# juicedata/juicefs

Measured on AMD Instinct MI355X. Metric: device-resident GiB/s (de)compress, 4 MiB blocks, LZ4+Zstd, 1/2/4/8 MI355X, higher is better.
Workload: dtype u8; 1 GPU; LZ4 decompress, 4096x4MiB blocks already in HBM (BASELINE configs[1]); blocks_per_gpu=4096, block_bytes=4194304, class=T, compressed_bytes_per_gpu=8570049795, parallelism=1 process(es), one per GPU, blocks sharded, no collective

## Files before the change

### juicefs_amd/csrc/lz4_decode.hip

```cpp
#include <hip/hip_runtime.h>
#include <stdint.h>

#include "jfs_internal.h"
#include "lz4_put16.h"
#include "lz4_tailpack.h"
#include "wave.cuh"

namespace jfs {
namespace lz4d {

constexpr int P = 32;
constexpr int CW = 64 * P;
constexpr int CWIN = CW + 80;
constexpr int R = 4096;
constexpr int RMASK = R - 1;
constexpr int SEG = 128;
constexpr int TMAX = CW / 3 + 2;
constexpr int TCAP = 448 < TMAX ? 448 : TMAX;
#ifndef JFS_DIAG
#define JFS_DIAG 0
#endif
enum : unsigned {
    D_SKIP_ZERO = 1,
    D_SKIP_LIT = 2,
    D_SKIP_FAR = 4,
    D_SKIP_SUBST = 8,
    D_SKIP_NEAR = 16,
    D_PARSEONLY = 32,
    D_NOCOPY = 64,
};
constexpr unsigned DIAG = JFS_DIAG;
constexpr uint32_t STOP = 0x80000000u;
constexpr uint32_t NONE = 0xFFFFFFFFu;
constexpr int KEXT = 64;
constexpr int FLUSH_T = 1024;
constexpr int LMAX = 64;
constexpr int BSPAN = 2048;
static_assert(BSPAN + FLUSH_T + 128 <= R, "ring must hold the unflushed tail plus one batch");
static_assert(R - BSPAN >= LMAX + 16, "far sources must lie below the flushed prefix");
static_assert(R == (int)TP_RING && LMAX <= (int)TP_LEN_MAX, "tail_pack field widths (lz4_tailpack.h)");

#ifdef JFS_PROF
#define NPROF 20
__device__ uint64_t g_prof[NPROF];
struct Prof {
    uint64_t t, acc[NPROF];
    __device__ void start() {
        t = __builtin_amdgcn_s_memtime();
        for (int i = 0; i < NPROF; i++) acc[i] = 0;
    }
    __device__ void stamp(int k) {
        uint64_t x = __builtin_amdgcn_s_memtime();
        acc[k] += x - t;
        t = x;
    }
    __device__ void flush_out() {
        if (__lane_id() == 0)
            for (int i = 0; i < NPROF; i++) atomicAdd((unsigned long long *)&g_prof[i], acc[i]);
    }
};
#define PSTAMP(k) pr.stamp(k)
#define PCOUNT(k, n) (pr.acc[k] += (n))
#define PROF_ARG , Prof &pr
#define PROF_PASS , pr
#else
#define PSTAMP(k)
#define PCOUNT(k, n)
#define PROF_ARG
#define PROF_PASS
#endif

enum { W_NONE = 0, W_WIN = 1, W_SER = 2, W_BUG = 3 };
struct Meta {
    int32_t kind, wbase, cbase;
    uint32_t T, efin;
};
struct Ctl {
    int32_t done, restart, rip;
    int32_t step;
};

struct Smem {
    alignas(16) uint8_t ring[R];
    alignas(16) uint8_t cwin[2][CWIN];
    alignas(16) uint16_t tab[2][TCAP];
    Meta meta[2];
    Ctl ctl;
};

struct Ctx {
    const gc_u8 *src;
    g_u8 *dst;
    int32_t n;
    int32_t cap;
    int32_t F;
    int32_t Fw;
    uint32_t dmis;
    int32_t cbase;
    int32_t bug;
    uint8_t *cw;
    uint32_t cwoff;
    uint16_t *tab;
};

typedef uint32_t u32x4 __attribute__((ext_vector_type(4), aligned(4)));
typedef uint32_t u32x2 __attribute__((ext_vector_type(2), aligned(4)));
typedef JFS_GLOBAL const u32x4 gc_x4;
typedef JFS_GLOBAL const u32x2 gc_x2;

__device__ __forceinline__ uint32_t slot(const Ctx &c, int32_t pos) { return (uint32_t)(pos + (int32_t)c.dmis) & RMASK; }

template <bool UNDER>
__device__ __forceinline__ void far_load(const Ctx &c, uintptr_t a, uint32_t &d0, uint32_t &d1, uint32_t &d2,
                                         uint32_t &d3, uint32_t &d4, uint32_t &d5) {
    const uintptr_t b = a & ~(uintptr_t)3, lo = (uintptr_t)c.dst & ~(uintptr_t)3;
    const bool under = UNDER && b < lo;
    const gc_x4 *q = (const gc_x4 *)(under ? lo : b);
    const u32x4 v = q[0];
    const u32x2 w = *(const gc_x2 *)(q + 1);
    d0 = v.x; d1 = v.y; d2 = v.z; d3 = v.w; d4 = w.x; d5 = w.y;
    if (under) { d5 = d4; d4 = d3; d3 = d2; d2 = d1; d1 = d0; d0 = 0; }
}

__device__ __forceinline__ uint32_t cb(const Smem &s, const Ctx &c, int32_t p) {
    int32_t r = p - c.cbase;
    if ((uint32_t)r < (uint32_t)CWIN) return c.cw[r];
    return (p >= 0 && p < c.n) ? c.src[p] : 0u;
}

__device__ __forceinline__ void stage_window(Smem &s, Ctx &c, int32_t wbase) {
    const int l = lane_id();
    const uint32_t mis = (uint32_t)(((uintptr_t)c.src + (uint32_t)wbase) & 15u);
    c.cbase = wbase - (int32_t)mis;
    constexpr int NCH = (CWIN / 16 + 63) / 64;
    uint4 v[NCH];
#pragma unroll
    for (int j = 0; j < NCH; ++j) {
        const int k = l + 64 * j;
        const int32_t p = c.cbase + 16 * k;
        v[j] = make_uint4(0, 0, 0, 0);
        if (k < CWIN / 16 && p < c.n) v[j] = *(const gc_u4 *)(c.src + p);
    }
#pragma unroll
    for (int j = 0; j < NCH; ++j) {
        const int k = l + 64 * j;
        if (k < CWIN / 16) *(uint4 *)(c.cw + 16 * k) = v[j];
    }
    if (c.cbase < 0 || c.cbase + CWIN > c.n) {
        for (int k = l; k < CWIN; k += 64) {
            int32_t p = c.cbase + k;
            if (p >= c.n || p < 0) c.cw[k] = 0;
        }
    }
}

struct Tok {
    int32_t nxt;
    int32_t ll;
    int32_t ml;
    int32_t off;
    int32_t lit;
    int32_t llx;
};

__device__ __forceinline__ Tok parse_tok(const Smem &s, const Ctx &c, int32_t p) {
    Tok t;
    const int32_t n = c.n;
    t.ll = t.ml = t.off = t.lit = t.llx = 0;
    if (p > n - 18) { t.nxt = (int32_t)(STOP | (uint32_t)p); return t; }
    uint32_t tb = cb(s, c, p);
    int32_t q = p + 1;
    int32_t ll = (int32_t)(tb >> 4);
    if (ll == 15) {
        t.llx = 1;
        int k = 0;
        uint32_t sv;
        do {
            sv = cb(s, c, q);
            q++;
            ll += (int32_t)sv;
            if (q >= n - 15 || ++k > KEXT) { t.nxt = (int32_t)(STOP | (uint32_t)p); return t; }
        } while (sv == 255);
        if (q + ll > n - 32) { t.nxt = (int32_t)(STOP | (uint32_t)p); return t; }
    }
    t.lit = q;
    t.ll = ll;
    q += ll;
    t.off = (int32_t)(cb(s, c, q) | (cb(s, c, q + 1) << 8));
    q += 2;
    int32_t ml = (int32_t)(tb & 15);
    if (ml == 15) {
        int k = 0;
        uint32_t sv;
        do {
            sv = cb(s, c, q);
            q++;
            ml += (int32_t)sv;
            if (q >= n - 4 || ++k > KEXT) { t.nxt = (int32_t)(STOP | (uint32_t)p); return t; }
        } while (sv == 255);
    }
    t.ml = ml + 4;
    t.nxt = q;
    return t;
}

struct FTok {
    int32_t nxt, lit;
    uint32_t ll, ml, off, llx;
    bool slow, stop;
};

__device__ __forceinline__ uint32_t w8(const Ctx &c, int32_t r) { return c.cw[r < CWIN - 1 ? r : CWIN - 1]; }

__device__ __forceinline__ FTok parse_fast(const Smem &s, const Ctx &c, int32_t p) {
    FTok t;
    const int32_t n = c.n, b0 = c.cbase;
    const int32_t r = p - b0;
    const uint32_t tb = w8(c, r), e1 = w8(c, r + 1);
    const bool llx = (tb >> 4) == 15;
    int32_t q = r + 1 + (llx ? 1 : 0);
    t.ll = (tb >> 4) + (llx ? e1 : 0u);
    bool slow = llx && e1 == 255;
    bool stop = p > n - 18;
    stop |= llx && (b0 + q >= n - 15 || b0 + q + (int32_t)t.ll > n - 32);
    t.lit = b0 + q;
    q += (int32_t)t.ll;
    slow |= q + 3 > CWIN;
    const uint32_t o0 = w8(c, q), o1 = w8(c, q + 1), e2 = w8(c, q + 2);
    q += 2;
    const bool mlx = (tb & 15) == 15;
    t.ml = (tb & 15) + (mlx ? e2 : 0u) + 4;
    q += mlx ? 1 : 0;
    slow |= mlx && e2 == 255;
    stop |= mlx && b0 + q >= n - 4;
    t.off = o0 | (o1 << 8);
    t.llx = llx ? 1u : 0u;
    t.nxt = b0 + q;
    t.slow = slow;
    t.stop = stop;
    return t;
}

__device__ __forceinline__ void flush(Smem &s, Ctx &c, int32_t to) {
    const int l = lane_id();
    int32_t F = c.F;
    if (to <= F) return;
    int32_t a = F + (int32_t)((16u - ((c.dmis + (uint32_t)F) & 15u)) & 15u);
    if (a > to) a = to;
    if (l < a - F) c.dst[F + l] = s.ring[slot(c, F + l)];
    int32_t b = a + ((to - a) & ~15);
    for (int32_t x = a + 16 * l; x < b; x += 1024) {
        uint4 v = *(const uint4 *)(s.ring + slot(c, x));
        *(g_u4 *)(c.dst + x) = v;
    }
    if (l < to - b) c.dst[b + l] = s.ring[slot(c, b + l)];
    c.F = to;
}

__device__ __forceinline__ void flush_to_line(Smem &s, Ctx &c, int32_t hi) {
    int32_t to = (int32_t)(((uint32_t)hi + c.dmis) & ~127u) - (int32_t)c.dmis;
    if (to > c.F) flush(s, c, to);
}

__device__ __forceinline__ uint32_t out_byte(const Smem &s, const Ctx &c, int32_t x, int32_t ringfloor) {
    if (x >= ringfloor) return s.ring[slot(c, x)];
    return c.dst[x];
}

__device__ __forceinline__ void need_flushed(Ctx &c, int32_t lim) {
    if (lim > c.Fw) {
        wait_vm();
        c.Fw = c.F;
    }
}

constexpr int32_t LIT_DIRECT = 2 * R;
__device__ __forceinline__ void direct_lit(Smem &s, Ctx &c, int32_t srcpos, int32_t op, int32_t body) {
    const int l = lane_id();
    flush(s, c, op);
    const gc_u8 *sp = c.src + srcpos - op;
    int32_t x = op;
    const int32_t ha = (int32_t)((16u - (((uint32_t)(uintptr_t)(c.dst + x)) & 15u)) & 15u);
    if (l < ha) c.dst[x + l] = sp[x + l];
    x += ha;
    for (; x + 4096 <= body; x += 4096) {
        u32x4 v[4];
        uint32_t w[4];
        const uint32_t sh = (uint32_t)((uintptr_t)(sp + x) & 3u);
#pragma unroll
        for (int j = 0; j < 4; ++j) {
            const uintptr_t a = (uintptr_t)(sp + x + 1024 * j + 16 * l) & ~(uintptr_t)3;
            v[j] = *(const gc_x4 *)a;
            w[j] = *(const gc_u32 *)(a + 16);
        }
#pragma unroll
        for (int j = 0; j < 4; ++j) {
            uint4 o;
            o.x = __builtin_amdgcn_alignbyte(v[j].y, v[j].x, sh);
            o.y = __builtin_amdgcn_alignbyte(v[j].z, v[j].y, sh);
            o.z = __builtin_amdgcn_alignbyte(v[j].w, v[j].z, sh);
            o.w = __builtin_amdgcn_alignbyte(w[j], v[j].w, sh);
            *(g_u4 *)(c.dst + x + 1024 * j + 16 * l) = o;
        }
    }
    for (; x < body; x += 64)
        if (x + l < body) c.dst[x + l] = sp[x + l];
    c.F = body;
}

__device__ __forceinline__ void coop_lit(Smem &s, Ctx &c, int32_t srcpos, int32_t op, int32_t len) {
    int l = lane_id();
    asm volatile("" : "+v"(l));
    if (len >= LIT_DIRECT) {
        const int32_t body = op + len - R;
        direct_lit(s, c, srcpos, op, body);
        srcpos += body - op;
        len -= body - op;
        op = body;
    }
    for (int32_t k = 0; k < len; k += 64) {
        if (op + k - c.F >= FLUSH_T) flush_to_line(s, c, op + k);
        int32_t i = k + l;
        if (i < len) s.ring[slot(c, op + i)] = cb(s, c, srcpos + i);
    }
}

__device__ __forceinline__ int32_t direct_fill(Smem &s, Ctx &c, int32_t op, int32_t off, int32_t len) {
    const int l = lane_id();
    const int32_t body = op + len - R;
    flush(s, c, op);
    const uint32_t amis = (uint32_t)(uintptr_t)(c.dst + op) & 15u;
    const int32_t x0 = op + (int32_t)((16u - amis) & 15u);
    uint32_t q[4] = {0, 0, 0, 0};
#pragma unroll
    for (int b = 0; b < 16; ++b) {
        const uint32_t v = s.ring[slot(c, op - off + (int32_t)(((uint32_t)(x0 - op) + (uint32_t)b) % (uint32_t)off))];
        q[b >> 2] |= v << (8 * (b & 3));
    }
    const uint4 chunk = make_uint4(q[0], q[1], q[2], q[3]);
    if (op + l < x0) c.dst[op + l] = s.ring[slot(c, op - off + (l % off))];
    int32_t x = x0;
    for (; x + 4096 <= body; x += 4096) {
#pragma unroll
        for (int j = 0; j < 4; ++j) *(g_u4 *)(c.dst + x + 1024 * j + 16 * l) = chunk;
    }
    for (; x + 16 <= body; x += 1024)
        if (x + 16 * l + 16 <= body) *(g_u4 *)(c.dst + x + 16 * l) = chunk;
    const int32_t xe = x0 + ((body - x0) & ~15);
    if (xe + l < body) c.dst[xe + l] = (uint8_t)(q[l >> 2 & 3] >> (8 * (l & 3)));
    if (l < 16) {
        const int32_t y = body - 16 + l;
        s.ring[slot(c, y)] = s.ring[slot(c, op - off + (int32_t)((uint32_t)(y - op) % (uint32_t)off))];
    }
    c.F = body;
    return body;
}

__device__ __forceinline__ void coop_match(Smem &s, Ctx &c, int32_t op, int32_t off, int32_t len) {
    int l = lane_id();
    asm volatile("" : "+v"(l));
    if (len >= LIT_DIRECT && off > 0 && off <= 16 && (16 % off) == 0) {
        const int32_t b = direct_fill(s, c, op, off, len);
        len -= b - op;
        op = b;
    }
    int32_t m = 0, step = 0;
    if (off > 0 && off < 64) { m = l % off; step = 64 % off; }
    for (int32_t k = 0; k < len; k += 64) {
        int32_t hi = op + k;
        if (hi - c.F >= FLUSH_T) flush_to_line(s, c, hi);
        int32_t ringfloor = hi + 64 - R;
        int32_t i = k + l;
        uint32_t v = 0;
        int32_t x = 0;
        if (off > 0) x = (off >= 64) ? op - off + i : op - off + m;
// ... 124 lines not shown
    cpy = op + length;
    if (cpy > cap - 12 && cpy > cap - 5) goto err;
    coop_match(s, c, op, offset, (int32_t)length);
    op = (int32_t)cpy;
    st.ip = ip;
    st.op = op;
    return SER_CONT;
err:
    st.ip = ip;
    st.ret = -ip - 1;
    return SER_ERR;
}

__device__ __forceinline__ uint32_t lomask(int32_t k) {
    k = k < 0 ? 0 : k;
    return k >= 4 ? 0xFFFFFFFFu : ((1u << (8 * k)) - 1u);
}

__device__ __forceinline__ void lds_or(uint8_t *ring, uint32_t a, uint32_t v) {
    __hip_atomic_fetch_or(reinterpret_cast<uint32_t *>(ring) + (a >> 2), v, __ATOMIC_RELAXED,
                          __HIP_MEMORY_SCOPE_WORKGROUP);
}
__device__ __forceinline__ void lds_or_at(uint32_t *p, uint32_t v) {
    __hip_atomic_fetch_or(p, v, __ATOMIC_RELAXED, __HIP_MEMORY_SCOPE_WORKGROUP);
}

template <bool WRAP>
__device__ __forceinline__ void put16(Smem &s, uint32_t da, int32_t m, uint32_t w0, uint32_t w1, uint32_t w2,
                                      uint32_t w3, uint32_t w4) {
    uint8_t *ring = s.ring;
    const Put16Masks k = put16_masks(da & 3u, (uint32_t)m);
    if constexpr (WRAP) {
        const uint32_t D0 = da & ~3u;
        lds_or(ring, D0, w0 & k.k[0]);
        lds_or(ring, (D0 + 4) & RMASK, w1 & k.k[1]);
        lds_or(ring, (D0 + 8) & RMASK, w2 & k.k[2]);
        lds_or(ring, (D0 + 12) & RMASK, w3 & k.k[3]);
        lds_or(ring, (D0 + 16) & RMASK, w4 & k.k[4]);
    } else {
        uint32_t *p = reinterpret_cast<uint32_t *>(ring) + (da >> 2);
        lds_or_at(p, w0 & k.k[0]);
        lds_or_at(p + 1, w1 & k.k[1]);
        lds_or_at(p + 2, w2 & k.k[2]);
        lds_or_at(p + 3, w3 & k.k[3]);
        lds_or_at(p + 4, w4 & k.k[4]);
    }
}

template <bool WRAP>
__device__ __forceinline__ void zero_span(Smem &s, const Ctx &c, int32_t O0, int32_t O1) {
    const int l = lane_id();
    const uint32_t a = slot(c, O0), h = a & 3u;
    if (l == 0 && h)
        __hip_atomic_fetch_and(reinterpret_cast<uint32_t *>(s.ring) + (a >> 2), lomask((int32_t)h), __ATOMIC_RELAXED,
                               __HIP_MEMORY_SCOPE_WORKGROUP);
    if constexpr (WRAP) {
        const int32_t A = O0 + (int32_t)((4u - h) & 3u);
        for (int32_t x = A + 4 * l; x < O1; x += 256) *(uint32_t *)(s.ring + slot(c, x)) = 0u;
    } else {
        const uint32_t e = a + (uint32_t)(O1 - O0);
        for (uint32_t x = ((a + 3u) & ~3u) + 4u * (uint32_t)l; x < e; x += 256) *(uint32_t *)(s.ring + x) = 0u;
    }
}

template <bool RING, bool WRAP>
__device__ __forceinline__ void copy16(Smem &s, uint32_t sa, uint32_t da, int32_t m) {
    const uint8_t *lds = (const uint8_t *)&s;
    const uint32_t ha = da & 3u;
    const uint32_t sb = RING ? (sa - ha) & RMASK : sa - ha, S0 = sb & ~3u, sh = sb & 3u;
    uint32_t r[6];
    if (RING && __ballot(S0 > (uint32_t)(R - 24))) {
#pragma unroll
        for (int j = 0; j < 6; ++j) r[j] = *(const uint32_t *)(lds + ((S0 + 4 * j) & RMASK));
    } else {
#pragma unroll
        for (int j = 0; j < 6; ++j) r[j] = *(const uint32_t *)(lds + S0 + 4 * j);
    }
    put16<WRAP>(s, da, m, __builtin_amdgcn_alignbyte(r[1], r[0], sh), __builtin_amdgcn_alignbyte(r[2], r[1], sh),
                __builtin_amdgcn_alignbyte(r[3], r[2], sh), __builtin_amdgcn_alignbyte(r[4], r[3], sh),
                __builtin_amdgcn_alignbyte(r[5], r[4], sh));
}


template <bool WRAP>
__device__ __forceinline__ void wave_near(Smem &s, uint32_t ds, uint32_t ss, int32_t len) {
    const int l = lane_id();
    const int32_t D = (int32_t)((ds - ss) & RMASK);
    const int32_t step = D < 64 ? D : 64;
    if (!WRAP && ss + (uint32_t)len <= (uint32_t)R) {
        const int32_t back = (int32_t)ss - (int32_t)ds;
        uint8_t *d = s.ring + ds + l;
        for (int32_t left = len; left > 0; left -= step, d += step)
            if (l < (left < step ? left : step)) d[0] = d[back];
        return;
    }
    for (int32_t k = 0; k < len; k += step) {
        const int32_t i = k + l;
        if (l < step && i < len) s.ring[(ds + (uint32_t)i) & RMASK] = s.ring[(ds + (uint32_t)(i - D)) & RMASK];
    }
}
__device__ __forceinline__ void wave_lit(Smem &s, const Ctx &c, int32_t op, uint32_t litr, int32_t from, int32_t len) {
    const int l = lane_id();
    for (int32_t k = from; k < len; k += 64) {
        const int32_t i = k + l;
        if (i < len) s.ring[slot(c, op + i)] = c.cw[litr + (uint32_t)i];
    }
}

template <bool WRAP>
__device__ __forceinline__ void batch(Smem &s, Ctx &c, bool act, int32_t o, uint32_t ll, uint32_t ml, uint32_t off,
                                      uint32_t litr, int32_t O0, int32_t O1 PROF_ARG) {
    const int32_t hz = O1 + 4 - R;
    asm volatile("" : "+v"(o));
    PCOUNT(14, 1);
    if (O0 - c.F >= FLUSH_T) flush_to_line(s, c, O0);
    if constexpr (!(DIAG & D_SKIP_ZERO)) zero_span<WRAP>(s, c, O0, O1);
    const int32_t ms = o + (int32_t)ll, msrc = ms - (int32_t)off;
    const uint32_t sbias = c.dmis - (((uint32_t)O0 + c.dmis) & ~(uint32_t)RMASK);
    auto dslot = [&](int32_t pos) -> uint32_t { return WRAP ? slot(c, pos) : (uint32_t)pos + sbias; };
    const bool hasm = act && ml > 0;
    const bool zero = hasm && off == 0;
    const bool far = hasm && off != 0 && msrc < hz;
    if (__ballot(far) && hz + LMAX > c.Fw) {
        wait_vm();
        c.Fw = c.F;
        if (hz + LMAX > c.Fw) c.bug = 4;
    }
    uint32_t fd0 = 0, fd1 = 0, fd2 = 0, fd3 = 0, fd4 = 0, fd5 = 0;
    const uint32_t fha = slot(c, ms) & 3u;
    if (__ballot(far)) {
        if (__ballot(far && msrc < 4)) {
            if (far) far_load<true>(c, (uintptr_t)(c.dst + msrc) - fha, fd0, fd1, fd2, fd3, fd4, fd5);
        } else {
            if (far) far_load<false>(c, (uintptr_t)(c.dst + msrc) - fha, fd0, fd1, fd2, fd3, fd4, fd5);
        }
    }
    for (uint32_t k = 0; !(DIAG & D_SKIP_LIT) && __ballot(act && k < ll); k += 16) {
        PCOUNT(16, 1);
        if (act && k < ll) {
            const int32_t m = ll - k < 16u ? (int32_t)(ll - k) : 16;
            copy16<false, WRAP>(s, c.cwoff + litr + k, dslot(o + (int32_t)k), m);
        }
    }
    PSTAMP(4);
    if (!(DIAG & D_SKIP_FAR) && __ballot(far)) {
        for (uint32_t k = 0; __ballot(far && k < ml); k += 16) {
            PCOUNT(17, 1);
            if (far && k < ml) {
                const int32_t m = ml - k < 16u ? (int32_t)(ml - k) : 16;
                const uint32_t da = dslot(ms + (int32_t)k);
                const uint32_t sh = (uint32_t)((uintptr_t)(c.dst + msrc + (int32_t)k) - fha) & 3u;
                put16<WRAP>(s, da, m, __builtin_amdgcn_alignbyte(fd1, fd0, sh),
                            __builtin_amdgcn_alignbyte(fd2, fd1, sh), __builtin_amdgcn_alignbyte(fd3, fd2, sh),
                            __builtin_amdgcn_alignbyte(fd4, fd3, sh), __builtin_amdgcn_alignbyte(fd5, fd4, sh));
            }
            const bool more = far && k + 16 < ml;
            if (__ballot(more)) {
                if (more)
                    far_load<false>(c, (uintptr_t)(c.dst + msrc + (int32_t)k + 16) - fha, fd0, fd1, fd2, fd3, fd4, fd5);
            }
        }
    }
    PSTAMP(5);
    bool pend = hasm && !far && !zero;
    int32_t src = msrc;
    const uint64_t am = __ballot(act);
    const int first = am ? (int)__builtin_ctzll(am) : 0;
    const uint32_t key = act ? (uint32_t)ms : (lane_id() < first ? 0u : 0xFFFFFFFFu);
    bool litsrc = false;
    {
        const uint32_t mek = pend ? (uint32_t)(ms + (int32_t)ml) : 0u;
        const bool want = !(DIAG & D_SKIP_SUBST) && pend && off >= ml && src >= O0;
        if (__ballot(want)) {
            int lo = 0;
#pragma unroll
            for (int stp = 32; stp; stp >>= 1) {
                const uint32_t v = (uint32_t)__shfl((int)key, lo + stp, 64);
                lo = v <= (uint32_t)src ? lo + stp : lo;
            }
            const uint32_t vms = (uint32_t)__shfl((int)key, lo, 64);
            const uint32_t vme = (uint32_t)__shfl((int)mek, lo, 64);
            const int32_t voff = __shfl((int)off, lo, 64);
            const bool ok = want && vms <= (uint32_t)src && (uint32_t)(src + (int32_t)ml) <= vme && voff > 0 &&
                            src - voff >= hz;
            const uint32_t nms = (uint32_t)__shfl((int)key, lo + 1 < 64 ? lo + 1 : 63, 64);
            litsrc = want && vms <= (uint32_t)src && (uint32_t)src >= vme && lo < 63 &&
                     (uint32_t)(src + (int32_t)ml) <= nms;
            src = ok ? src - voff : src;
        }
    }
    int32_t pos = ms, rem = (int32_t)ml, D = ms - src;
    const int32_t send = src + (int32_t)ml < ms ? src + (int32_t)ml : ms;
    if (!(DIAG & D_SKIP_NEAR)) {
        PCOUNT(18, 1);
        const bool go = pend && (send <= O0 || litsrc);
        if (__ballot(go)) {
            PCOUNT(15, 1);
            if (go) {
                const int32_t m = rem < 16 ? (rem < D ? rem : D) : (D < 16 ? D : 16);
                copy16<true, WRAP>(s, slot(c, pos - D), dslot(pos), m);
                pos += m;
                rem -= m;
                if (rem <= 0) pend = false;
            }
        }
        const uint32_t tw = tail_pack(dslot(pos), slot(c, pos - D), (uint32_t)rem, (uint32_t)D);
        for (uint64_t pmk = __ballot(pend); pmk;) {
            const int j = (int)__builtin_ctzll(pmk);
            pmk &= ~(1ull << j);
            PCOUNT(19, 1);
            const uint32_t w = readlane(tw, j);
            if (tail_direct(w)) {
                if ((uint32_t)lane_id() < tail_rem(w)) s.ring[tail_ds(w) + lane_id()] = s.ring[tail_ss(w) + lane_id()];
            } else {
                wave_near<WRAP>(s, tail_ds(w), tail_ss(w), (int32_t)tail_rem(w));
            }
        }
    }
    PSTAMP(6);
}

__device__ __forceinline__ uint32_t copy_tokens(Smem &s, Ctx &c, uint32_t T, int32_t op0, int32_t *end_op,
                                                int32_t *bad_ip PROF_ARG) {
    const int l = lane_id();
    int32_t op = op0;
    const int32_t cap = c.cap;
    if constexpr ((DIAG & D_PARSEONLY) != 0) {
        *end_op = op0;
        return T;
    }
    for (uint32_t g0 = 0; g0 < T; g0 += 64) {
        const uint32_t n0 = T - g0 < 64u ? T - g0 : 64u;
        const bool in0 = (uint32_t)l < n0;
        const int32_t p = c.cbase + (in0 ? (int32_t)c.tab[g0 + l] : 0);
        FTok t = parse_fast(s, c, p);
        const bool sl = in0 && t.slow;
        if (__ballot(sl)) {
            if (sl) {
                const Tok u = parse_tok(s, c, p);
                t.lit = u.lit;
                t.ll = (uint32_t)u.ll;
                t.ml = (uint32_t)u.ml;
                t.off = (uint32_t)u.off;
                t.llx = (uint32_t)u.llx;
            }
        }
        const uint32_t ll = in0 ? t.ll : 0u, ml = in0 ? t.ml : 0u, off = t.off;
        const uint32_t litr = (uint32_t)(t.lit - c.cbase);
        const uint32_t len = ll + ml;
        const uint32_t incl = dpp_scan_add(len);
        const int32_t o = op + (int32_t)(incl - len);
        const int32_t om = o + (int32_t)ll;
        const bool bad = in0 && ((t.llx && om > cap - 32) || (om + (int32_t)ml >= cap - 64) || ((int32_t)off > om));
        const uint64_t bm = __ballot(bad);
        const uint32_t n = bm ? (uint32_t)__builtin_ctzll(bm) : n0;
        const bool in = (uint32_t)l < n;
        const int32_t endo = o + (int32_t)len;
        const bool lng = in && (ll > (uint32_t)LMAX || ml > (uint32_t)LMAX);
        PSTAMP(2);
        uint32_t j = 0;
        while (j < n) {
            const int32_t oj = (int32_t)readlane((uint32_t)o, (int)j);
            if (readlane(lng ? 1u : 0u, (int)j)) {
                const uint32_t jll = readlane(ll, (int)j), jml = readlane(ml, (int)j), joff = readlane(off, (int)j);
                const uint32_t jlit = readlane(litr, (int)j);
                coop_lit(s, c, c.cbase + (int32_t)jlit, oj, (int32_t)jll);
                coop_match(s, c, oj + (int32_t)jll, (int32_t)joff, (int32_t)jml);
                PSTAMP(7);
                j++;
                continue;
            }
            const bool ok = (uint32_t)l >= j && in && !lng && endo - oj <= BSPAN;
            const uint64_t stop = __ballot(!ok) & (~0ull << j);
            const uint32_t e = stop ? (uint32_t)__builtin_ctzll(stop) : 64u;
            const uint32_t eb = e > n ? n : e;
            const bool act = (uint32_t)l >= j && (uint32_t)l < eb;
            const int32_t O1 = (int32_t)readlane((uint32_t)endo, (int)eb - 1);
            PSTAMP(3);
            if constexpr (!(DIAG & D_NOCOPY)) {
                if (slot(c, oj) + (uint32_t)(O1 - oj) + 20u <= (uint32_t)R)
                    batch<false>(s, c, act, o, ll, ml, off, litr, oj, O1 PROF_PASS);
                else
                    batch<true>(s, c, act, o, ll, ml, off, litr, oj, O1 PROF_PASS);
            }
            j = eb;
        }
        if (bm) {
            *bad_ip = (int32_t)readlane((uint32_t)p, (int)n);
            *end_op = (int32_t)readlane((uint32_t)o, (int)n);
            return g0 + n;
        }
        op += (int32_t)readlane(incl, 63);
    }
    *end_op = op;
    return T;
}

static_assert(SEG == 128, "segment bit sets are two u64 per lane");
constexpr int SW = 64 * SEG;
constexpr int SPRE = 32;
constexpr int SEG_BUDGET = 64;
constexpr int SEG_MIN = 4;

__device__ __noinline__ uint32_t g_next_exact(const Ctx &c, int32_t p) {
    const int32_t n = c.n;
    if (p > n - 18) return STOP | (uint32_t)p;
    const uint32_t tb = c.src[p];
    int32_t q = p + 1;
    int32_t ll = (int32_t)(tb >> 4);
    if (ll == 15) {
        int k = 0;
        uint32_t sv;
        do {
            sv = c.src[q];
            q++;
            ll += (int32_t)sv;
            if (q >= n - 15 || ++k > KEXT) return STOP | (uint32_t)p;
        } while (sv == 255);
        if (q + ll > n - 32) return STOP | (uint32_t)p;
    }
    q += ll + 2;
    if ((tb & 15u) == 15u) {
        int k = 0;
        uint32_t sv;
        do {
            sv = c.src[q];
            q++;
            if (q >= n - 4 || ++k > KEXT) return STOP | (uint32_t)p;
        } while (sv == 255);
    }
    return (uint32_t)q;
}

__device__ __forceinline__ uint32_t g_step(const Ctx &c, int32_t p, bool act) {
    const int32_t n = c.n;
    const uint32_t edge = (uint32_t)(p > n - 18);
    const uint32_t up = (uint32_t)p;
    const uint32_t tb = c.src[edge ? 0u : up], e1 = c.src[edge ? 0u : up + 1u];
    const uint32_t hi = tb >> 4;
    const uint32_t llx = (uint32_t)(hi == 15u);
    const uint32_t L = llx ? 15u + e1 : hi;
    const uint32_t lstop = llx & ((uint32_t)(p + 2 >= n - 15) | (uint32_t)(p + 2 + (int32_t)L > n - 32));
    const uint32_t q = up + 3u + llx + L;
    const uint32_t e2 = c.src[(edge | lstop) ? 0u : q];
    const uint32_t mlx = (uint32_t)((tb & 15u) == 15u);
    uint32_t x = q + mlx;
    const uint32_t slow = (uint32_t)act & (edge ^ 1u) & (lstop ^ 1u) & ((llx & (uint32_t)(e1 == 255u)) | (mlx & (uint32_t)(e2 == 255u)));
    x = (edge | lstop | (mlx & (uint32_t)((int32_t)x >= n - 4))) ? (STOP | up) : x;
    if (__ballot(slow)) {
        if (slow) x = g_next_exact(c, p);
    }
    return x;
}

__device__ __forceinline__ bool tbit2(uint64_t a0, uint64_t a1, uint32_t d) {
    return (((d < 64u ? a0 : a1) >> (d & 63u)) & 1ull) != 0;
}
__device__ __forceinline__ void sbit2(uint64_t &a0, uint64_t &a1, uint32_t d) {
    const uint64_t m = 1ull << (d & 63u);
    a0 |= d < 64u ? m : 0ull;
    a1 |= d < 64u ? 0ull : m;
}
__device__ __forceinline__ uint64_t from_lo(uint32_t d) { return d < 64u ? (~0ull << (d & 63u)) : 0ull; }
__device__ __forceinline__ uint64_t from_hi(uint32_t d) { return d < 64u ? ~0ull : (~0ull << (d & 63u)); }

struct SegWalk {
    int32_t base, plo, phi;
    int32_t q;
    uint32_t cur;
    uint32_t sx, ex;
    uint64_t vs0, vs1;
    uint64_t vt0, vt1;
    uint64_t vp0, vp1;
    bool mv;
    int phase;
    bool round;
    int steps, rounds;

    __device__ __forceinline__ void start(int32_t b) {
        const int l = lane_id();
        base = b;
        plo = b + l * SEG;
        phi = plo + SEG;
        cur = l == 0 ? (uint32_t)b : (uint32_t)(plo - SPRE);
        q = (int32_t)cur;
        vs0 = vs1 = vt0 = vt1 = vp0 = vp1 = 0;
        sx = ex = 0;
        mv = true;
        phase = 0;
        round = false;
        steps = rounds = 0;
    }

    __device__ __forceinline__ bool advance(Ctx &c, int budget PROF_ARG) {
        if (phase == 0) {
            for (; budget > 0 && __ballot(mv); --budget) {
                PCOUNT(11, 1);
                if (mv) {
                    const uint32_t x = g_step(c, q, true);
                    const bool stop = (x & STOP) != 0;
                    if (!stop && q >= plo) sbit2(vs0, vs1, (uint32_t)(q - plo));
                    const bool out = stop || (int32_t)x >= phi;
                    sx = out ? x : sx;
                    mv = !out;
                    q = (int32_t)x;
                }
                if (++steps > SEG + SPRE) { c.bug = 6; phase = 2; return true; }
            }
            if (budget == 0) return false;
            vt0 = vs0;
            vt1 = vs1;
            ex = sx;
            phase = 1;
            round = true;
        }
        while (phase == 1 && budget > 0) {
            if (round) {
                const uint32_t In = dpp_shift_up(ex, (uint32_t)base);
                const bool ch = In != cur;
                if (!__ballot(ch)) { phase = 2; break; }
                if (++rounds > 64) { c.bug = 3; phase = 2; break; }
                PCOUNT(12, 1);
                mv = false;
                if (ch) {
                    cur = In;
                    const uint32_t d = In - (uint32_t)plo;
                    if ((In & STOP) || (int32_t)In >= phi) {
                        vt0 = vt1 = 0;
                        ex = In;
                    } else if (tbit2(vs0, vs1, d)) {
                        vt0 = vs0 & from_lo(d);
                        vt1 = vs1 & from_hi(d);
                        ex = sx;
                    } else {
                        mv = true;
                    }
                }
                q = (int32_t)In;
                vp0 = vp1 = 0;
                steps = 0;
                round = false;
            }
            for (; budget > 0 && __ballot(mv); --budget) {
                PCOUNT(13, 1);
                if (mv) {
                    const uint32_t d = (uint32_t)(q - plo);
                    const bool join = tbit2(vs0, vs1, d);
                    const uint32_t x = g_step(c, q, !join);
                    const bool stop = !join && (x & STOP) != 0;
                    if (!join && !stop) sbit2(vp0, vp1, d);
                    const bool out = join || stop || (int32_t)x >= phi;
                    if (out) {
                        vt0 = vp0 | (join ? vs0 & from_lo(d) : 0ull);
                        vt1 = vp1 | (join ? vs1 & from_hi(d) : 0ull);
                        ex = join ? sx : x;
                    }
                    mv = !out;
                    q = (int32_t)x;
                }
                if (++steps > SEG + 1) { c.bug = 7; phase = 2; return true; }
            }
            if (!__ballot(mv)) round = true;
        }
        return phase == 2;
    }
};

__device__ __forceinline__ uint32_t span_dword(uint64_t vt0, uint64_t vt1, int32_t k) {
    const int src = (k >> 2) & 63;
    const uint32_t d0 = (uint32_t)__shfl((int)(uint32_t)vt0, src, 64);
    const uint32_t d1 = (uint32_t)__shfl((int)(uint32_t)(vt0 >> 32), src, 64);
    const uint32_t d2 = (uint32_t)__shfl((int)(uint32_t)vt1, src, 64);
    const uint32_t d3 = (uint32_t)__shfl((int)(uint32_t)(vt1 >> 32), src, 64);
    const uint32_t j = (uint32_t)k & 3u;
    const uint32_t v = j == 0 ? d0 : j == 1 ? d1 : j == 2 ? d2 : d3;
    return (k >= 0 && k < 4 * 64) ? v : 0u;
}

struct Span {
    uint64_t v0, v1;
    int32_t base;
    uint32_t exit;
};

__device__ __forceinline__ void parse_window_seg(Smem &s, Ctx &c, int32_t wbase, const Span &sp, uint32_t *T_out,
                                                 uint32_t *efin_out PROF_ARG) {
    static_assert(P == 32, "a window lane covers one dword of the span bit set");
    const int l = lane_id();
    stage_window(s, c, wbase);
    const int32_t cbase = c.cbase;
    PCOUNT(10, 1);
    __builtin_amdgcn_wave_barrier();
    PSTAMP(0);
    const int32_t send = sp.base + SW;
    const int32_t wend = cbase + CW < send ? cbase + CW : send;
    const int32_t o = cbase - sp.base + 32 * l;
    const int32_t K = o >> 5;
    const uint32_t lo = span_dword(sp.v0, sp.v1, K), hi = span_dword(sp.v0, sp.v1, K + 1);
    uint32_t field = __builtin_amdgcn_alignbit(hi, lo, (uint32_t)o & 31u);
    const int32_t plo = cbase + 32 * l;
    const int32_t a = wbase - plo, b = wend - plo;
    const uint32_t ma = a <= 0 ? 0xFFFFFFFFu : a >= 32 ? 0u : (0xFFFFFFFFu << a);
    const uint32_t mb = b >= 32 ? 0xFFFFFFFFu : b <= 0 ? 0u : ((1u << b) - 1u);
    field &= ma & mb;
    PSTAMP(1);
    const uint32_t cnt = (uint32_t)__builtin_popcount(field);
    const uint32_t cinc = dpp_scan_add(cnt);
    const uint32_t tall = readlane(cinc, 63);
    *T_out = tall < (uint32_t)TCAP ? tall : (uint32_t)TCAP;
    uint32_t ex = 0;
    {
        uint32_t idx = cinc - cnt;
        uint32_t v = field;
        while (__ballot(v != 0)) {
            if (v) {
                const uint32_t bb = (uint32_t)__builtin_ctz(v);
                if (idx < (uint32_t)TCAP) c.tab[idx] = (uint16_t)((uint32_t)l * P + bb);
                else if (idx == (uint32_t)TCAP) ex = (uint32_t)plo + bb;
                idx++;
                v &= v - 1;
            }
        }
    }
    if (tall > (uint32_t)TCAP) {
        const uint64_t hit = __ballot(cinc - cnt <= (uint32_t)TCAP && (uint32_t)TCAP < cinc);
        *efin_out = readlane(ex, (int)__builtin_ctzll(hit));
    } else if (wend >= send) {
        *efin_out = sp.exit;
    } else {
        const int32_t d = wend - sp.base - l * SEG;
        const uint32_t dd = d < 0 ? 0u : (uint32_t)d;
        const uint64_t m0 = d >= SEG ? 0ull : sp.v0 & from_lo(dd), m1 = d >= SEG ? 0ull : sp.v1 & from_hi(dd);
        const uint64_t any = __ballot((m0 | m1) != 0ull);
        if (any) {
            const int f = (int)__builtin_ctzll(any);
            const uint32_t bit = m0 ? (uint32_t)__builtin_ctzll(m0) : 64u + (uint32_t)__builtin_ctzll(m1 | (1ull << 63));
            *efin_out = (uint32_t)sp.base + (uint32_t)(f * SEG) + readlane(bit, f);
        } else {
            *efin_out = sp.exit;
        }
    }
    PSTAMP(2);
}

__device__ __forceinline__ void wg_sync() { asm volatile("s_waitcnt lgkmcnt(0)\n\ts_barrier" ::: "memory"); }

__device__ __forceinline__ void use_buffer(Smem &s, Ctx &c, int buf) {
    c.cw = s.cwin[buf];
    c.cwoff = (uint32_t)((const uint8_t *)s.cwin[buf] - (const uint8_t *)&s);
    c.tab = s.tab[buf];
}

__device__ __forceinline__ void parser_wave(Smem &s, Ctx &c PROF_ARG) {
    int32_t pip = 0;
    bool pstop = false;
    Span sp;
    sp.v0 = sp.v1 = 0;
    sp.base = 0;
    sp.exit = 0;
    bool spv = false;
    bool nxt = false;
    SegWalk wk;
    wk.start(0);
    for (uint32_t k = 0;; ++k) {
        const int buf = (int)(k & 1u);
        Meta m;
        m.kind = W_NONE;
        m.wbase = pip;
        m.cbase = 0;
        m.T = 0;
        m.efin = 0;
        if (!pstop) {
            if (pip < c.n - 64) {
                use_buffer(s, c, buf);
                uint32_t T, efin;
                if (!spv || pip >= sp.base + SW) {
                    if (!(spv && nxt && wk.base == pip)) wk.start(pip);
                    wk.advance(c, 1 << 20 PROF_PASS);
                    PSTAMP(1);
                    sp.v0 = wk.vt0;
                    sp.v1 = wk.vt1;
                    sp.base = pip;
                    sp.exit = readlane(wk.ex, 63);
                    spv = true;
                    nxt = !(sp.exit & STOP) && !c.bug;
                    if (nxt) wk.start((int32_t)sp.exit);
                }
                parse_window_seg(s, c, pip, sp, &T, &efin PROF_PASS);
                if (nxt) {
                    bool fin = wk.advance(c, SEG_MIN PROF_PASS);
                    for (int g = SEG_MIN; !fin && g < SEG_BUDGET; g += 2) {
                        if (__hip_atomic_load(&s.ctl.step, __ATOMIC_RELAXED, __HIP_MEMORY_SCOPE_WORKGROUP) >= (int32_t)k)
                            break;
                        fin = wk.advance(c, 2 PROF_PASS);
                    }
                }
                PSTAMP(1);
                m.kind = c.bug ? W_BUG : W_WIN;
                m.cbase = c.cbase;
                m.T = T;
                m.efin = efin;
                if ((efin & STOP) || c.bug) pstop = true;
                else pip = (int32_t)efin;
            } else {
                m.kind = W_SER;
                pstop = true;
            }
        }
        if (lane_id() == 0) s.meta[buf] = m;
        wg_sync();
        const int32_t done = (int32_t)uniform((uint32_t)s.ctl.done), restart = (int32_t)uniform((uint32_t)s.ctl.restart),
                      rip = (int32_t)uniform((uint32_t)s.ctl.rip);
        wg_sync();
        PSTAMP(9);
        if (done) break;
        if (restart) {
            pip = rip;
            pstop = false;
            spv = false;
            nxt = false;
        }
    }
}

template <bool PREFIX>
__device__ __forceinline__ void copier_wave(Smem &s, Ctx &c, int32_t *retp, int32_t want PROF_ARG) {
    __builtin_amdgcn_s_setprio(1);
    Ser st;
    st.ip = 0;
    st.op = 0;
    st.fast = c.cap >= 64;
    st.ret = 0;
    bool skip = false;
    int32_t result = INT32_MIN;
    int64_t nser = 0;
    if (lane_id() == 0) __hip_atomic_store(&s.ctl.step, -1, __ATOMIC_RELAXED, __HIP_MEMORY_SCOPE_WORKGROUP);
    for (uint32_t k = 0;; ++k) {
        int32_t done = 0, restart = 0, rip = 0;
        if (k > 0 && !skip) {
            const int buf = (int)((k - 1) & 1u);
            Meta m;
            m.kind = (int32_t)uniform((uint32_t)s.meta[buf].kind);
            m.wbase = (int32_t)uniform((uint32_t)s.meta[buf].wbase);
            m.cbase = (int32_t)uniform((uint32_t)s.meta[buf].cbase);
            m.T = uniform(s.meta[buf].T);
            m.efin = uniform(s.meta[buf].efin);
            bool ser = false;
            if (m.kind == W_BUG || m.kind == W_NONE || m.wbase != st.ip) {
                c.bug |= 8;
            } else if (m.kind == W_WIN && st.fast && st.ip < c.n - 64 && st.op < c.cap - 128) {
                use_buffer(s, c, buf);
                c.cbase = m.cbase;
                int32_t end_op = st.op, bad_ip = 0;
                const uint32_t dn = m.T > 0 ? copy_tokens(s, c, m.T, st.op, &end_op, &bad_ip PROF_PASS) : 0u;
                st.op = end_op;
                if (dn < m.T) {
                    st.ip = bad_ip;
                    ser = true;
                } else {
                    st.ip = (int32_t)(m.efin & ~STOP);
                    ser = (m.efin & STOP) != 0;
                }
                if constexpr (PREFIX) {
                    if (st.op >= want) {
                        ser = false;
                        flush(s, c, st.op);
                        result = want;
                        done = 1;
                    }
                }
            } else {
                ser = true;
            }
            if (ser && !c.bug) {
                c.cbase = 0x3fffffff;
                for (;;) {
                    const int status = ser_seq(s, c, st);
                    if (status != SER_CONT) {
                        if (status == SER_DONE) flush(s, c, st.op);
                        result = st.ret;
                        if constexpr (PREFIX) result = st.ret > want ? want : st.ret;
                        done = 1;
                        break;
                    }
                    if constexpr (PREFIX) {
                        if (st.op >= want) {
                            flush(s, c, st.op);
                            result = want;
                            done = 1;
                            break;
                        }
                    }
                    if (++nser > (int64_t)c.n + 64) { c.bug |= 16; break; }
                    if (st.fast && st.ip < c.n - 64 && st.op < c.cap - 128) {
                        restart = 1;
                        rip = st.ip;
                        break;
                    }
                }
                PSTAMP(7);
            }
            if (c.bug) {
                done = 1;
                restart = 0;
                result = INT32_MIN;
            }
        }
        if (k > (uint32_t)c.n + 64) {
            done = 1;
            result = INT32_MIN;
        }
        if (lane_id() == 0) {
            s.ctl.done = done;
            s.ctl.restart = restart;
            s.ctl.rip = rip;
            __hip_atomic_store(&s.ctl.step, (int32_t)k, __ATOMIC_RELAXED, __HIP_MEMORY_SCOPE_WORKGROUP);
        }
        wg_sync();
        wg_sync();
        PSTAMP(8);
        if (done) break;
        skip = restart != 0;
    }
    if (lane_id() == 0) *retp = result;
}

#define JFS_LZ4_ATTR __attribute__((amdgpu_num_sgpr(80), amdgpu_waves_per_eu(8)))
template <bool PREFIX, class... WANT>
__global__ __launch_bounds__(128) JFS_LZ4_ATTR void lz4_decode_kernel(const jfs_dev_block *__restrict__ blocks, int nblk,
                                                        int32_t *__restrict__ ret,
                                                        const int32_t *__restrict__ lens,
                                                        const int32_t *__restrict__ todo, WANT... wantp) {
    static_assert(sizeof...(WANT) == (PREFIX ? 1 : 0), "the prefix instantiation takes want, the full one does not");
    __shared__ Smem s;
    const int b = blockIdx.x;
    if (b >= nblk) return;
    if (todo && !todo[b]) return;
    const int wave = (int)uniform(threadIdx.x >> 6);
    jfs_dev_block d = ((const gc_blk *)blocks)[b];
    Ctx c;
    c.src = (const gc_u8 *)d.src;
    c.dst = (g_u8 *)d.dst;
    c.n = lens ? lens[b] : d.src_len;
    if (lens && c.n < 0) {
        if (threadIdx.x == 64) ret[b] = JFS_CHAIN_FAILED;
        return;
    }
    c.cap = d.dst_cap;
    c.F = 0;
    c.Fw = 0;
    c.dmis = (uint32_t)((uintptr_t)d.dst & 15u);
    c.cbase = 0x3fffffff;
    c.bug = 0;
    use_buffer(s, c, 0);
#ifdef JFS_PROF
    Prof pr;
    pr.start();
#endif
    int32_t early = 1, result = 0;
    if (d.src == nullptr || c.n < 0 || c.cap < 0) result = -1;
    else if (c.cap == 0) result = (c.n == 1 && c.src[0] == 0) ? 0 : -1;
    else if (c.n == 0) result = -1;
    else early = 0;
    if (early) {
        if (wave == 1 && lane_id() == 0) ret[b] = result;
        return;
    }
    int32_t want = 0;
    if constexpr (PREFIX) {
        want = (int32_t)uniform((uint32_t)(wantp, ...)[b]);
        if (want <= 0) {
            if (wave == 1 && lane_id() == 0) ret[b] = 0;
            return;
        }
        if (want > c.cap) want = c.cap;
    }
    if (wave == 0) parser_wave(s, c PROF_PASS);
    else copier_wave<PREFIX>(s, c, ret + b, want PROF_PASS);
#ifdef JFS_PROF
    pr.flush_out();
#endif
}

}
}

#ifndef JFS_LZ4_DECODE_PREFIX_TU
#ifdef JFS_PROF
extern "C" int jfs_prof_read(uint64_t *out) {
    return hipMemcpyFromSymbol(out, HIP_SYMBOL(jfs::lz4d::g_prof), sizeof(uint64_t) * NPROF) == hipSuccess ? 0 : -1;
}
extern "C" int jfs_prof_reset() {
    uint64_t z[NPROF] = {0};
    return hipMemcpyToSymbol(HIP_SYMBOL(jfs::lz4d::g_prof), z, sizeof(z)) == hipSuccess ? 0 : -1;
}
#endif

extern "C" int jfs_launch_lz4_decode(const jfs_dev_block *d_blocks, int nblk, int32_t *d_ret, hipStream_t stream) {
    return jfs_launch_lz4_decode_lens(d_blocks, nblk, d_ret, nullptr, stream);
}

extern "C" int jfs_launch_lz4_decode_lens(const jfs_dev_block *d_blocks, int nblk, int32_t *d_ret, const int32_t *d_lens,
                                          hipStream_t stream) {
    if (nblk <= 0) return 0;
    hipLaunchKernelGGL(jfs::lz4d::lz4_decode_kernel<false>, dim3(nblk), dim3(128), 0, stream, d_blocks, nblk, d_ret,
                       d_lens, (const int32_t *)nullptr);
    return hipGetLastError() == hipSuccess ? 0 : -1;
}

extern "C" int jfs_launch_lz4_decode_todo(const jfs_dev_block *d_blocks, int nblk, int32_t *d_ret, const int32_t *d_todo,
                                          hipStream_t stream) {
    if (nblk <= 0) return 0;
    hipLaunchKernelGGL(jfs::lz4d::lz4_decode_kernel<false>, dim3(nblk), dim3(128), 0, stream, d_blocks, nblk, d_ret,
                       (const int32_t *)nullptr, d_todo);
    return hipGetLastError() == hipSuccess ? 0 : -1;
}

#else
extern "C" int jfs_launch_lz4_decode_prefix(const jfs_dev_block *d_blocks, int nblk, int32_t *d_ret,
                                            const int32_t *d_want, const int32_t *d_todo, hipStream_t stream) {
    if (nblk <= 0) return 0;
    hipLaunchKernelGGL((jfs::lz4d::lz4_decode_kernel<true, const int32_t *>), dim3(nblk), dim3(128), 0, stream,
                       d_blocks, nblk, d_ret, (const int32_t *)nullptr, d_todo, d_want);
    return hipGetLastError() == hipSuccess ? 0 : -1;
}
#endif
```

Measured before the change: 491.5 GiB/s.

## Speculatively defer match-length byte check in LZ4 segment walk to overlap loads

Restructures the per-lane token walk used to find segment boundaries so that the match-length extension byte (e2) is fetched in one iteration and checked in the next. The next token's loads can then issue without waiting on the e2 load. If the deferred byte turns out to be 255, the step is redone with the exact parser; this adds redo iterations and more state, and an asm barrier keeps the loads grouped. Profiling counters for the first-window latency are also added, but they only compile under JFS_PROF.

```diff
diff --git a/juicefs_amd/csrc/lz4_decode.hip b/juicefs_amd/csrc/lz4_decode.hip
--- a/juicefs_amd/csrc/lz4_decode.hip
+++ b/juicefs_amd/csrc/lz4_decode.hip
@@ -4,6 +4,7 @@
 #include "jfs_internal.h"
 #include "lz4_put16.h"
 #include "lz4_tailpack.h"
+#include "lz4_walkstep.h"
 #include "wave.cuh"
 
 namespace jfs {
@@ -41,17 +42,18 @@
 static_assert(R == (int)TP_RING && LMAX <= (int)TP_LEN_MAX, "tail_pack field widths (lz4_tailpack.h)");
 
 #ifdef JFS_PROF
-#define NPROF 20
+#define NPROF 30
 __device__ uint64_t g_prof[NPROF];
 struct Prof {
-    uint64_t t, acc[NPROF];
+    uint64_t t, last, acc[NPROF];
     __device__ void start() {
         t = __builtin_amdgcn_s_memtime();
         for (int i = 0; i < NPROF; i++) acc[i] = 0;
     }
     __device__ void stamp(int k) {
         uint64_t x = __builtin_amdgcn_s_memtime();
-        acc[k] += x - t;
+        last = x - t;
+        acc[k] += last;
         t = x;
     }
     __device__ void flush_out() {
@@ -61,16 +63,27 @@
 };
 #define PSTAMP(k) pr.stamp(k)
 #define PCOUNT(k, n) (pr.acc[k] += (n))
+#define PFIRST(...) __VA_ARGS__
+#define PWALK(kind)                                                        \
+    do {                                                                   \
+        const uint64_t re_ = __ballot((kind) == WS_REDONE);                \
+        pr.acc[26] += (uint64_t)__popcll(re_);                             \
+        pr.acc[27] += re_ != 0;                                            \
+        pr.acc[28] += (uint64_t)__popcll(__ballot((kind) == WS_ARRIVED)); \
+    } while (0)
 #define PROF_ARG , Prof &pr
 #define PROF_PASS , pr
 #else
 #define PSTAMP(k)
 #define PCOUNT(k, n)
+#define PFIRST(...)
+#define PWALK(kind) (void)(kind)
 #define PROF_ARG
 #define PROF_PASS
 #endif
 
 enum { W_NONE = 0, W_WIN = 1, W_SER = 2, W_BUG = 3 };
+constexpr int32_t W_PFIRST = 16;
 struct Meta {
     int32_t kind, wbase, cbase;
     uint32_t T, efin;
@@ -801,67 +814,11 @@
 constexpr int SEG_BUDGET = 64;
 constexpr int SEG_MIN = 4;
 
+static_assert(WS_STOP == STOP && WS_KEXT == KEXT, "lz4_walkstep.h restates the parser's constants");
 __device__ __noinline__ uint32_t g_next_exact(const Ctx &c, int32_t p) {
-    const int32_t n = c.n;
-    if (p > n - 18) return STOP | (uint32_t)p;
-    const uint32_t tb = c.src[p];
-    int32_t q = p + 1;
-    int32_t ll = (int32_t)(tb >> 4);
-    if (ll == 15) {
-        int k = 0;
-        uint32_t sv;
-        do {
-            sv = c.src[q];
-            q++;
-            ll += (int32_t)sv;
-            if (q >= n - 15 || ++k > KEXT) return STOP | (uint32_t)p;
-        } while (sv == 255);
-        if (q + ll > n - 32) return STOP | (uint32_t)p;
-    }
-    q += ll + 2;
-    if ((tb & 15u) == 15u) {
-        int k = 0;
-        uint32_t sv;
-        do {
-            sv = c.src[q];
-            q++;
-            if (q >= n - 4 || ++k > KEXT) return STOP | (uint32_t)p;
-        } while (sv == 255);
-    }
-    return (uint32_t)q;
-}
-
-__device__ __forceinline__ uint32_t g_step(const Ctx &c, int32_t p, bool act) {
-    const int32_t n = c.n;
-    const uint32_t edge = (uint32_t)(p > n - 18);
-    const uint32_t up = (uint32_t)p;
-    const uint32_t tb = c.src[edge ? 0u : up], e1 = c.src[edge ? 0u : up + 1u];
-    const uint32_t hi = tb >> 4;
-    const uint32_t llx = (uint32_t)(hi == 15u);
-    const uint32_t L = llx ? 15u + e1 : hi;
-    const uint32_t lstop = llx & ((uint32_t)(p + 2 >= n - 15) | (uint32_t)(p + 2 + (int32_t)L > n - 32));
-    const uint32_t q = up + 3u + llx + L;
-    const uint32_t e2 = c.src[(edge | lstop) ? 0u : q];
-    const uint32_t mlx = (uint32_t)((tb & 15u) == 15u);
-    uint32_t x = q + mlx;
-    const uint32_t slow = (uint32_t)act & (edge ^ 1u) & (lstop ^ 1u) & ((llx & (uint32_t)(e1 == 255u)) | (mlx & (uint32_t)(e2 == 255u)));
-    x = (edge | lstop | (mlx & (uint32_t)((int32_t)x >= n - 4))) ? (STOP | up) : x;
-    if (__ballot(slow)) {
-        if (slow) x = g_next_exact(c, p);
-    }
-    return x;
-}
-
-__device__ __forceinline__ bool tbit2(uint64_t a0, uint64_t a1, uint32_t d) {
-    return (((d < 64u ? a0 : a1) >> (d & 63u)) & 1ull) != 0;
-}
-__device__ __forceinline__ void sbit2(uint64_t &a0, uint64_t &a1, uint32_t d) {
-    const uint64_t m = 1ull << (d & 63u);
-    a0 |= d < 64u ? m : 0ull;
-    a1 |= d < 64u ? 0ull : m;
-}
-__device__ __forceinline__ uint64_t from_lo(uint32_t d) { return d < 64u ? (~0ull << (d & 63u)) : 0ull; }
-__device__ __forceinline__ uint64_t from_hi(uint32_t d) { return d < 64u ? ~0ull : (~0ull << (d & 63u)); }
+    return ws_next_exact([&](uint32_t i) { return (uint32_t)c.src[i]; }, c.n, p);
+}
+
 
 struct SegWalk {
     int32_t base, plo, phi;
@@ -872,6 +829,8 @@
     uint64_t vt0, vt1;
     uint64_t vp0, vp1;
     bool mv;
+    uint32_t pe2;
+    bool pend;
     int phase;
     bool round;
     int steps, rounds;
@@ -886,24 +845,22 @@
         vs0 = vs1 = vt0 = vt1 = vp0 = vp1 = 0;
         sx = ex = 0;
         mv = true;
+        pe2 = 0;
+        pend = false;
         phase = 0;
         round = false;
         steps = rounds = 0;
     }
 
     __device__ __forceinline__ bool advance(Ctx &c, int budget PROF_ARG) {
+        const auto fetch = [&](uint32_t i) { return (uint32_t)c.src[i]; };
+        const auto exact = [&](int32_t p) { return g_next_exact(c, p); };
         if (phase == 0) {
             for (; budget > 0 && __ballot(mv); --budget) {
                 PCOUNT(11, 1);
-                if (mv) {
-                    const uint32_t x = g_step(c, q, true);
-                    const bool stop = (x & STOP) != 0;
-                    if (!stop && q >= plo) sbit2(vs0, vs1, (uint32_t)(q - plo));
-                    const bool out = stop || (int32_t)x >= phi;
-                    sx = out ? x : sx;
-                    mv = !out;
-                    q = (int32_t)x;
-                }
+                int kind = WS_STEPPED;
+                if (mv) kind = ws_spec_iter(*this, fetch, exact, c.n);
+                PWALK(kind);
                 if (++steps > SEG + SPRE) { c.bug = 6; phase = 2; return true; }
             }
             if (budget == 0) return false;
@@ -942,21 +899,9 @@
             }
             for (; budget > 0 && __ballot(mv); --budget) {
                 PCOUNT(13, 1);
-                if (mv) {
-                    const uint32_t d = (uint32_t)(q - plo);
-                    const bool join = tbit2(vs0, vs1, d);
-                    const uint32_t x = g_step(c, q, !join);
-                    const bool stop = !join && (x & STOP) != 0;
-                    if (!join && !stop) sbit2(vp0, vp1, d);
-                    const bool out = join || stop || (int32_t)x >= phi;
-                    if (out) {
-                        vt0 = vp0 | (join ? vs0 & from_lo(d) : 0ull);
-                        vt1 = vp1 | (join ? vs1 & from_hi(d) : 0ull);
-                        ex = join ? sx : x;
-                    }
-                    mv = !out;
-                    q = (int32_t)x;
-                }
+                int kind = WS_STEPPED;
+                if (mv) kind = ws_fix_iter(*this, fetch, exact, c.n);
+                PWALK(kind);
                 if (++steps > SEG + 1) { c.bug = 7; phase = 2; return true; }
             }
             if (!__ballot(mv)) round = true;
@@ -1069,14 +1014,18 @@
         m.cbase = 0;
         m.T = 0;
         m.efin = 0;
+        PFIRST(bool pfirst = false);
         if (!pstop) {
             if (pip < c.n - 64) {
                 use_buffer(s, c, buf);
                 uint32_t T, efin;
                 if (!spv || pip >= sp.base + SW) {
                     if (!(spv && nxt && wk.base == pip)) wk.start(pip);
+                    PFIRST(const uint64_t it0 = pr.acc[11] + pr.acc[13]; pfirst = true);
                     wk.advance(c, 1 << 20 PROF_PASS);
                     PSTAMP(1);
+                    PFIRST(const uint64_t its = pr.acc[11] + pr.acc[13] - it0; pr.acc[22] += 1; pr.acc[23] += its;
+                           pr.acc[24] += pr.last; pr.acc[25] += its == 0);
                     sp.v0 = wk.vt0;
                     sp.v1 = wk.vt1;
                     sp.base = pip;
@@ -1096,6 +1045,7 @@
                 }
                 PSTAMP(1);
                 m.kind = c.bug ? W_BUG : W_WIN;
+                PFIRST(if (pfirst && !c.bug) m.kind |= W_PFIRST);
                 m.cbase = c.cbase;
                 m.T = T;
                 m.efin = efin;
@@ -1112,6 +1062,7 @@
                       rip = (int32_t)uniform((uint32_t)s.ctl.rip);
         wg_sync();
         PSTAMP(9);
+        PFIRST(if (pfirst) pr.acc[21] += pr.last);
         if (done) break;
         if (restart) {
             pip = rip;
@@ -1133,6 +1084,7 @@
     bool skip = false;
     int32_t result = INT32_MIN;
     int64_t nser = 0;
+    PFIRST(uint64_t wait8 = 0);
     if (lane_id() == 0) __hip_atomic_store(&s.ctl.step, -1, __ATOMIC_RELAXED, __HIP_MEMORY_SCOPE_WORKGROUP);
     for (uint32_t k = 0;; ++k) {
         int32_t done = 0, restart = 0, rip = 0;
@@ -1140,6 +1092,7 @@
             const int buf = (int)((k - 1) & 1u);
             Meta m;
             m.kind = (int32_t)uniform((uint32_t)s.meta[buf].kind);
+            PFIRST(if (m.kind & W_PFIRST) pr.acc[20] += wait8; m.kind &= ~W_PFIRST);
             m.wbase = (int32_t)uniform((uint32_t)s.meta[buf].wbase);
             m.cbase = (int32_t)uniform((uint32_t)s.meta[buf].cbase);
             m.T = uniform(s.meta[buf].T);
@@ -1218,6 +1171,7 @@
         wg_sync();
         wg_sync();
         PSTAMP(8);
+        PFIRST(wait8 = pr.last);
         if (done) break;
         skip = restart != 0;
     }
diff --git a/juicefs_amd/csrc/lz4_walkstep.h b/juicefs_amd/csrc/lz4_walkstep.h
--- /dev/null
+++ b/juicefs_amd/csrc/lz4_walkstep.h
@@ -0,0 +1,150 @@
+#pragma once
+#include <stdint.h>
+
+#if defined(__HIPCC__)
+#define JFS_WALKSTEP_HD __host__ __device__ __forceinline__
+#else
+#define JFS_WALKSTEP_HD inline
+#endif
+
+namespace jfs {
+namespace lz4d {
+
+constexpr uint32_t WS_STOP = 0x80000000u;
+constexpr int WS_KEXT = 64;
+
+template <class F>
+JFS_WALKSTEP_HD uint32_t ws_next_exact(F fetch, int32_t n, int32_t p) {
+    if (p > n - 18) return WS_STOP | (uint32_t)p;
+    const uint32_t tb = fetch((uint32_t)p);
+    int32_t q = p + 1;
+    int32_t ll = (int32_t)(tb >> 4);
+    if (ll == 15) {
+        int k = 0;
+        uint32_t sv;
+        do {
+            sv = fetch((uint32_t)q);
+            q++;
+            ll += (int32_t)sv;
+            if (q >= n - 15 || ++k > WS_KEXT) return WS_STOP | (uint32_t)p;
+        } while (sv == 255);
+        if (q + ll > n - 32) return WS_STOP | (uint32_t)p;
+    }
+    q += ll + 2;
+    if ((tb & 15u) == 15u) {
+        int k = 0;
+        uint32_t sv;
+        do {
+            sv = fetch((uint32_t)q);
+            q++;
+            if (q >= n - 4 || ++k > WS_KEXT) return WS_STOP | (uint32_t)p;
+        } while (sv == 255);
+    }
+    return (uint32_t)q;
+}
+
+struct WsRound {
+    uint32_t x;
+    uint32_t q;
+    uint32_t halt;
+    uint32_t ext;
+    uint32_t mlx;
+};
+template <class F>
+JFS_WALKSTEP_HD WsRound ws_round(F fetch, int32_t n, int32_t p, uint32_t &pe2) {
+    const uint32_t edge = (uint32_t)(p > n - 18);
+    const uint32_t up = (uint32_t)p;
+    uint32_t tb = fetch(edge ? 0u : up), e1 = fetch(edge ? 0u : up + 1u);
+#if defined(__HIP_DEVICE_COMPILE__)
+    asm volatile("" : "+v"(tb), "+v"(e1), "+v"(pe2));
+#endif
+    const uint32_t hi = tb >> 4;
+    const uint32_t llx = (uint32_t)(hi == 15u);
+    const uint32_t L = llx ? 15u + e1 : hi;
+    const uint32_t lstop = llx & ((uint32_t)(p + 2 >= n - 15) | (uint32_t)(p + 2 + (int32_t)L > n - 32));
+    WsRound r;
+    r.q = up + 3u + llx + L;
+    r.mlx = (uint32_t)((tb & 15u) == 15u);
+    r.x = r.q + r.mlx;
+    r.halt = edge | lstop;
+    r.ext = (r.halt ^ 1u) & llx & (uint32_t)(e1 == 255u);
+    return r;
+}
+
+JFS_WALKSTEP_HD bool tbit2(uint64_t a0, uint64_t a1, uint32_t d) {
+    return (((d < 64u ? a0 : a1) >> (d & 63u)) & 1ull) != 0;
+}
+JFS_WALKSTEP_HD void sbit2(uint64_t &a0, uint64_t &a1, uint32_t d) {
+    const uint64_t m = 1ull << (d & 63u);
+    a0 |= d < 64u ? m : 0ull;
+    a1 |= d < 64u ? 0ull : m;
+}
+JFS_WALKSTEP_HD void pbit2(uint64_t &a0, uint64_t &a1, uint32_t d, bool on) {
+    const uint64_t m = 1ull << (d & 63u);
+    uint64_t &a = d < 64u ? a0 : a1;
+    a = on ? a | m : a & ~m;
+}
+JFS_WALKSTEP_HD uint64_t from_lo(uint32_t d) { return d < 64u ? (~0ull << (d & 63u)) : 0ull; }
+JFS_WALKSTEP_HD uint64_t from_hi(uint32_t d) { return d < 64u ? ~0ull : (~0ull << (d & 63u)); }
+
+enum { WS_STEPPED = 0, WS_REDONE = 1, WS_ARRIVED = 2 };
+
+template <class W, class F>
+JFS_WALKSTEP_HD uint32_t ws_take(W &w, uint32_t &pp, const WsRound &r, F fetch, int32_t n, bool *ext) {
+    const uint32_t last = r.mlx & (uint32_t)((int32_t)r.x >= n - 4);
+    const uint32_t pend = (r.halt ^ 1u) & (r.ext ^ 1u) & r.mlx & (last ^ 1u);
+    w.pe2 = fetch(pend ? r.q : 0u);
+    pp = (uint32_t)w.q;
+    w.pend = pend != 0;
+    *ext = r.ext != 0;
+    return (r.halt | last) ? (WS_STOP | (uint32_t)w.q) : r.x;
+}
+
+template <class W, class F, class X>
+JFS_WALKSTEP_HD int ws_spec_iter(W &w, F fetch, X exact, int32_t n) {
+    const WsRound r = ws_round(fetch, n, w.q, w.pe2);
+    const bool redo = w.pend && w.pe2 == 255u;
+    const bool arr = w.pend && !redo && w.q >= w.phi;
+    const int32_t at = redo ? (int32_t)w.sx : w.q;
+    uint32_t x = (uint32_t)w.q;
+    bool ex = redo;
+    if (redo || arr) w.pend = false;
+    else x = ws_take(w, w.sx, r, fetch, n, &ex);
+    if (ex) x = exact(at);
+    const bool stop = (x & WS_STOP) != 0;
+    if (!arr && at >= w.plo) pbit2(w.vs0, w.vs1, (uint32_t)(at - w.plo), !stop);
+    const bool out = stop || (!w.pend && (int32_t)x >= w.phi);
+    w.sx = out ? x : w.sx;
+    w.mv = !out;
+    w.q = (int32_t)x;
+    return redo ? WS_REDONE : arr ? WS_ARRIVED : WS_STEPPED;
+}
+
+template <class W, class F, class X>
+JFS_WALKSTEP_HD int ws_fix_iter(W &w, F fetch, X exact, int32_t n) {
+    const WsRound r = ws_round(fetch, n, w.q, w.pe2);
+    const bool redo = w.pend && w.pe2 == 255u;
+    const bool arr = w.pend && !redo && w.q >= w.phi;
+    const int32_t at = redo ? (int32_t)w.ex : w.q;
+    const uint32_t d = (uint32_t)(at - w.plo);
+    const bool join = !redo && !arr && tbit2(w.vs0, w.vs1, d);
+    uint32_t x = (uint32_t)w.q;
+    bool ex = redo;
+    if (redo || arr || join) w.pend = false;
+    else x = ws_take(w, w.ex, r, fetch, n, &ex);
+    if (ex) x = exact(at);
+    const bool stop = (x & WS_STOP) != 0;
+    if (!arr && !join) pbit2(w.vp0, w.vp1, d, !stop);
+    const bool out = join || stop || (!w.pend && (int32_t)x >= w.phi);
+    if (out) {
+        w.vt0 = w.vp0 | (join ? w.vs0 & from_lo(d) : 0ull);
+        w.vt1 = w.vp1 | (join ? w.vs1 & from_hi(d) : 0ull);
+        w.ex = join ? w.sx : x;
+    }
+    w.mv = !out;
+    w.q = (int32_t)x;
+    return redo ? WS_REDONE : arr ? WS_ARRIVED : WS_STEPPED;
+}
+
+}
+}
```

Measured after the change: 509.8 GiB/s, median of 6. +3.7%, better.
